# tobwei/APTAI

Measured on AMD Instinct MI355X. Metric: utterances/sec (10 s @ 16 kHz) train-step, higher is better.
Workload: dtype bf16

## Files before the change

### aptai_amd/csrc/gemm.hip

```cpp
#include <stdlib.h>

#include <mutex>
#include <set>
#include <type_traits>

#include "common.h"
#include "gemm_common.h"

using namespace aptai_gemm;

namespace {

#ifdef APTAI_STAMPS
__device__ unsigned long long g_stamps[4096 * 8];
#define APTAI_STAMP(slot)                                                                          \
    do {                                                                                           \
        if (threadIdx.x == 0 && blockIdx.x < 4096 && blockIdx.y == 0 && blockIdx.z == 0)           \
            g_stamps[blockIdx.x * 8 + (slot)] = wall_clock64();                                    \
    } while (0)
extern "C" int aptai_debug_read_stamps(void* host_out) {
    return hipMemcpyFromSymbol(host_out, HIP_SYMBOL(g_stamps), sizeof(g_stamps)) == hipSuccess ? 0 : 1;
}
#else
#define APTAI_STAMP(slot) do {} while (0)
#endif

void epi_trace(const GemmArgs& g, int tile) {
    static const bool on = getenv("APTAI_EPI_TRACE") != nullptr;
    if (!on) return;
    static std::mutex mu;
    static std::set<int> seen;
    const int w = g.flags | (g.out_pre ? EPX_PRE : 0) | (g.colscale_n > 0 ? EPX_CS : 0);
    std::lock_guard<std::mutex> lk(mu);
    if (!seen.insert(w).second) return;
    bool listed = false;
#define APTAI_EPI_CASE(W) listed = listed || (w == (W));
    APTAI_EPI_WORDS(APTAI_EPI_CASE)
#undef APTAI_EPI_CASE
    fprintf(stderr, "[aptai epi] flag word 0x%x (tile %d, %d x %d x %d): %s\n", w, tile, g.M, g.N, g.K, listed ? "compiled" : "RUN-TIME form");
}

template <bool A_KM, bool B_KM, bool OUT_F32, int BM_T = 128>
__device__ __forceinline__ void gemm_tile_body(GemmArgs g, const int bid, const int batch, const int split) {
    extern __shared__ __attribute__((aligned(16))) char smem[];
    APTAI_STAMP(0);
    const int tid = threadIdx.x;
    const int lane = tid & 63;
    const int wave = __builtin_amdgcn_readfirstlane(tid >> 6);
    const int wm = wave >> 1, wn = wave & 1;

    int tile_m, tile_n;
    raster2d(bid, g.tiles_m, g.tiles_n, g.raster_gm, tile_m, tile_n);
    constexpr int NI = BM_T / 32;
    constexpr int WM = BM_T / 2;
    constexpr int NA_IT = BM_T / 32;
    constexpr int A_BYTES_T = BM_T * BK * 2;
    constexpr int STAGE_T = A_BYTES_T + BN * BK * 2;
    constexpr int NPASS = BM_T / 16;
    static_assert(BM_T == 128 || (BM_T == 64 && !A_KM), "64-row tiles are built for K-contiguous A only");
    constexpr bool RING5 = A_KM && B_KM && BM_T == 128 && APTAI_GEMM_RING5;
    const int m0 = tile_m * BM_T, n0 = tile_n * BN;

    if (batch >= 0) {
        const int bo = batch / g.nb_inner, bi = batch % g.nb_inner;
        g.A += bo * g.sA[0] + bi * g.sA[1];
        g.B += bo * g.sB[0] + bi * g.sB[1];
        const long co = bo * g.sC[0] + bi * g.sC[1];
        g.C = (OUT_F32 && !(g.flags & APTAI_EPI_SPLIT_OUT)) ? (void*)((float*)g.C + co) : (void*)((bf16_t*)g.C + co);
        if (g.out_pre) g.out_pre += co;
        if (g.bias) g.bias += bo * g.sBias[0] + bi * g.sBias[1];
        if (g.residual) g.residual += bo * g.sR[0] + bi * g.sR[1];
        if (g.aux) g.aux += bo * g.sAux[0] + bi * g.sAux[1];
    }
    const int total_kt = g.K / BK;
    const int kt_begin = split * g.ktiles_per_split;
    int kt_end = kt_begin + g.ktiles_per_split;
    kt_end = kt_end < total_kt ? kt_end : total_kt;
    const int nk = kt_end - kt_begin;

    f32x4 acc[NI][4];
#pragma unroll
    for (int i = 0; i < NI; ++i)
#pragma unroll
        for (int j = 0; j < 4; ++j) acc[i][j] = (f32x4){0.f, 0.f, 0.f, 0.f};

    const int wave_base_tid = wave * 64;
    const bool wave_active = (m0 + wm * WM < g.M) && (n0 + wn * 64 < g.N);
    const bf16_t* pa[NA_IT];
    const bf16_t* pb[4];
    const long stepA = A_KM ? (long)BK * g.lda : (long)BK, stepB = B_KM ? (long)BK * g.ldb : (long)BK;
#pragma unroll
    for (int it = 0; it < NA_IT; ++it) pa[it] = stage_src<A_KM>(g.A, g.lda, m0, g.M, it, tid) + kt_begin * stepA;
#pragma unroll
    for (int it = 0; it < 4; ++it) pb[it] = stage_src<B_KM>(g.B, g.ldb, n0, g.N, it, tid) + kt_begin * stepB;
    auto stage = [&](char* buf) {
        char* dst = buf + wave_base_tid * 16;
#pragma unroll
        for (int it = 0; it < NA_IT; ++it) {
            __builtin_amdgcn_global_load_lds(GLB_PTR(pa[it]), LDS_PTR(dst + it * (NTHREADS * 16)), 16, 0, 0);
            pa[it] += stepA;
        }
#pragma unroll
        for (int it = 0; it < 4; ++it) {
            __builtin_amdgcn_global_load_lds(GLB_PTR(pb[it]), LDS_PTR(dst + A_BYTES_T + it * (NTHREADS * 16)), 16, 0, 0);
            pb[it] += stepB;
        }
    };
    if constexpr (RING5) {
        constexpr int HALF_T = RING_HALF_BYTES;
        const bf16_t* ha[2];
        const bf16_t* hb[2];
        const long hstepA = 32 * (long)g.lda, hstepB = 32 * (long)g.ldb;
#pragma unroll
        for (int it = 0; it < 2; ++it) {
            ha[it] = stage_src<true>(g.A, g.lda, m0, g.M, it, tid) + kt_begin * stepA;
            hb[it] = stage_src<true>(g.B, g.ldb, n0, g.N, it, tid) + kt_begin * stepB;
        }
        auto stage_half = [&](int slot) {
            char* dst = smem + slot * HALF_T + wave_base_tid * 16;
#pragma unroll
            for (int it = 0; it < 2; ++it) {
                __builtin_amdgcn_global_load_lds(GLB_PTR(ha[it]), LDS_PTR(dst + it * (NTHREADS * 16)), 16, 0, 0);
                ha[it] += hstepA;
            }
#pragma unroll
            for (int it = 0; it < 2; ++it) {
                __builtin_amdgcn_global_load_lds(GLB_PTR(hb[it]), LDS_PTR(dst + HALF_T / 2 + it * (NTHREADS * 16)), 16, 0, 0);
                hb[it] += hstepB;
            }
        };
        uint32_t frag_off[16];
        {
            const int gq = lane >> 4, li = lane & 15, qq = li >> 2, pp = li & 3;
            const int k_lo = gq * 8 + qq, k_hi = k_lo + 4;
            const int sub = (pp & 1) << 3;
#pragma unroll
            for (int f = 0; f < 8; ++f) {
                const int is_b = f >> 2, idx = f & 3;
                const int row_base = is_b ? wn * 64 + idx * 16 : wm * WM + idx * 16;
                const int ch = (row_base >> 3) + (pp >> 1);
                frag_off[2 * f] = (uint32_t)(is_b * (HALF_T / 2) + k_lo * 256 + ((ch ^ km_swz(k_lo)) << 4) + sub);
                frag_off[2 * f + 1] = (uint32_t)(is_b * (HALF_T / 2) + k_hi * 256 + ((ch ^ km_swz(k_hi)) << 4) + sub);
            }
        }
        const uint32_t ring_base = (uint32_t)(uintptr_t)(__attribute__((address_space(3))) const char*)smem;
        const int nh = 2 * nk;
        if (nh > 0) { stage_half(0); stage_half(1); }
        if (nh > 2) stage_half(2);
        int s0 = 0;
        for (int kt = 0; kt < nk; ++kt) {
            if (kt + 1 < nk) asm volatile("s_waitcnt vmcnt(4) lgkmcnt(0)" ::: "memory");
            else asm volatile("s_waitcnt vmcnt(0) lgkmcnt(0)" ::: "memory");
            __builtin_amdgcn_s_barrier();
            asm volatile("" ::: "memory");
            const int s1 = s0 + 1 >= 5 ? s0 - 4 : s0 + 1, s2 = s0 + 2 >= 5 ? s0 - 3 : s0 + 2, s3 = s0 + 3 >= 5 ? s0 - 2 : s0 + 3,
                      s4 = s0 + 4 >= 5 ? s0 - 1 : s0 + 4;
            if (2 * kt + 3 < nh) stage_half(s3);
            if (2 * kt + 4 < nh) stage_half(s4);
            if (wave_active) {
                short4v fr[2][16];
#pragma unroll
                for (int hh = 0; hh < 2; ++hh) {
                    const uint32_t base = ring_base + (uint32_t)((hh ? s1 : s0) * HALF_T);
#pragma unroll
                    for (int f = 0; f < 16; ++f)
                        asm volatile("ds_read_b64_tr_b16 %0, %1" : "=v"(fr[hh][f]) : "v"(base + frag_off[f]));
                }
#define APTAI_TIE8(h, o) "+v"(fr[h][o]), "+v"(fr[h][o + 1]), "+v"(fr[h][o + 2]), "+v"(fr[h][o + 3]), "+v"(fr[h][o + 4]), \
                         "+v"(fr[h][o + 5]), "+v"(fr[h][o + 6]), "+v"(fr[h][o + 7])
#pragma unroll
                for (int hh = 0; hh < 2; ++hh) {
                    if (hh == 0) asm volatile("s_waitcnt lgkmcnt(15)" : APTAI_TIE8(0, 0), APTAI_TIE8(0, 8));
                    else asm volatile("s_waitcnt lgkmcnt(0)" : APTAI_TIE8(1, 0), APTAI_TIE8(1, 8));
                    bf16x8 af[NI], bfr[4];
#pragma unroll
                    for (int i = 0; i < NI; ++i) {
                        const short4v lo4 = fr[hh][2 * i], hi4 = fr[hh][2 * i + 1];
                        af[i] = __builtin_bit_cast(bf16x8, (short8v){lo4[0], lo4[1], lo4[2], lo4[3], hi4[0], hi4[1], hi4[2], hi4[3]});
                    }
#pragma unroll
                    for (int j = 0; j < 4; ++j) {
                        const short4v lo4 = fr[hh][8 + 2 * j], hi4 = fr[hh][8 + 2 * j + 1];
                        bfr[j] = __builtin_bit_cast(bf16x8, (short8v){lo4[0], lo4[1], lo4[2], lo4[3], hi4[0], hi4[1], hi4[2], hi4[3]});
                    }
#pragma unroll
                    for (int i = 0; i < NI; ++i)
#pragma unroll
                        for (int j = 0; j < 4; ++j)
                            acc[i][j] = __builtin_amdgcn_mfma_f32_16x16x32_bf16(bfr[j], af[i], acc[i][j], 0, 0, 0);
                }
#undef APTAI_TIE8
            }
            s0 = s2;
        }
        asm volatile("s_waitcnt vmcnt(0) lgkmcnt(0)" ::: "memory");
        __syncthreads();
    } else {
    if (nk > 0) stage(smem);
    for (int kt = 0; kt < nk; ++kt) {
        asm volatile("s_waitcnt vmcnt(0)" ::: "memory");
        __syncthreads();
        const int cur = kt & 1;
        if (kt + 1 < nk) stage(smem + (cur ^ 1) * STAGE_T);
        const char* sa = smem + cur * STAGE_T;
        const char* sb = sa + A_BYTES_T;
        if (wave_active) {
            if constexpr (!A_KM && !B_KM && APTAI_GEMM_HOIST) {
                bf16x8 af[2][NI], bfr[2][4];
#pragma unroll
                for (int ks = 0; ks < 2; ++ks) {
#pragma unroll
                    for (int j = 0; j < 4; ++j) bfr[ks][j] = read_frag<B_KM>(sb, wn * 64 + j * 16, ks, lane);
#pragma unroll
                    for (int i = 0; i < NI; ++i) af[ks][i] = read_frag<A_KM>(sa, wm * WM + i * 16, ks, lane);
                }
                __builtin_amdgcn_sched_barrier(0);
#pragma unroll
                for (int ks = 0; ks < 2; ++ks)
#pragma unroll
                    for (int i = 0; i < NI; ++i)
#pragma unroll
                        for (int j = 0; j < 4; ++j)
                            acc[i][j] = __builtin_amdgcn_mfma_f32_16x16x32_bf16(bfr[ks][j], af[ks][i], acc[i][j], 0, 0, 0);
            } else if constexpr (BM_T == 64 && !A_KM && B_KM && APTAI_GEMM_M64_ASM) {
                short4v bl[2][4], bh[2][4];
                u32x4 aa[2][2];
#pragma unroll
                for (int ks = 0; ks < 2; ++ks) {
#pragma unroll
                    for (int j = 0; j < 4; ++j) read_frag_tr_asm(sb, wn * 64 + j * 16, ks, lane, bl[ks][j], bh[ks][j]);
#pragma unroll
                    for (int i = 0; i < 2; ++i) {
                        const int row = wm * WM + i * 16 + (lane & 15), q = ks * 4 + (lane >> 4);
                        const uint32_t addr = lds_u32(sa) + (uint32_t)(row * 128 + ((q ^ (row & 7)) << 4));
                        asm volatile("ds_read_b128 %0, %1" : "=v"(aa[ks][i]) : "v"(addr));
                    }
                }
#pragma unroll
                for (int ks = 0; ks < 2; ++ks) {
                    if (ks == 0)
                        asm volatile("s_waitcnt lgkmcnt(10)" : "+v"(bl[0][0]), "+v"(bl[0][1]), "+v"(bl[0][2]), "+v"(bl[0][3]), "+v"(bh[0][0]),
                                                               "+v"(bh[0][1]), "+v"(bh[0][2]), "+v"(bh[0][3]), "+v"(aa[0][0]), "+v"(aa[0][1]));
                    else
                        asm volatile("s_waitcnt lgkmcnt(0)" : "+v"(bl[1][0]), "+v"(bl[1][1]), "+v"(bl[1][2]), "+v"(bl[1][3]), "+v"(bh[1][0]),
                                                              "+v"(bh[1][1]), "+v"(bh[1][2]), "+v"(bh[1][3]), "+v"(aa[1][0]), "+v"(aa[1][1]));
#pragma unroll
                    for (int i = 0; i < 2; ++i)
#pragma unroll
                        for (int j = 0; j < 4; ++j)
                            acc[i][j] = __builtin_amdgcn_mfma_f32_16x16x32_bf16(combine_tr(bl[ks][j], bh[ks][j]),
                                                                                __builtin_bit_cast(bf16x8, aa[ks][i]), acc[i][j], 0, 0, 0);
                }
            } else {
#pragma unroll
                for (int ks = 0; ks < 2; ++ks) {
                    bf16x8 af[NI], bfr[4];
                    constexpr bool ASM_TR = BM_T == 128;
                    short4v tl[NI + 4], th[NI + 4];
#pragma unroll
                    for (int j = 0; j < 4; ++j) {
                        if constexpr (B_KM && ASM_TR) read_frag_tr_asm(sb, wn * 64 + j * 16, ks, lane, tl[NI + j], th[NI + j]);
                        else bfr[j] = read_frag<B_KM>(sb, wn * 64 + j * 16, ks, lane);
                    }
#pragma unroll
                    for (int i = 0; i < NI; ++i) {
                        if constexpr (A_KM && ASM_TR) read_frag_tr_asm(sa, wm * WM + i * 16, ks, lane, tl[i], th[i]);
                        else af[i] = read_frag<A_KM>(sa, wm * WM + i * 16, ks, lane);
                    }
                    if constexpr (B_KM && ASM_TR) {
                        asm volatile("s_waitcnt lgkmcnt(0)"
                                     : "+v"(tl[NI]), "+v"(tl[NI + 1]), "+v"(tl[NI + 2]), "+v"(tl[NI + 3]), "+v"(th[NI]), "+v"(th[NI + 1]),
                                       "+v"(th[NI + 2]), "+v"(th[NI + 3]));
#pragma unroll
                        for (int j = 0; j < 4; ++j) bfr[j] = combine_tr(tl[NI + j], th[NI + j]);
                    }
                    if constexpr (A_KM && ASM_TR) {
                        static_assert(!A_KM || NI == 4, "K-major A is built for 128-row tiles");
                        asm volatile("s_waitcnt lgkmcnt(0)"
                                     : "+v"(tl[0]), "+v"(tl[1]), "+v"(tl[2]), "+v"(tl[3]), "+v"(th[0]), "+v"(th[1]), "+v"(th[2]), "+v"(th[3]));
#pragma unroll
                        for (int i = 0; i < NI; ++i) af[i] = combine_tr(tl[i], th[i]);
                    }
#pragma unroll
                    for (int i = 0; i < NI; ++i)
#pragma unroll
                        for (int j = 0; j < 4; ++j)
                            acc[i][j] = __builtin_amdgcn_mfma_f32_16x16x32_bf16(bfr[j], af[i], acc[i][j], 0, 0, 0);
                }
            }
        }
    }
    }

    APTAI_STAMP(2);
    int tid_e = tid, lane_e = lane, m0_e = __builtin_amdgcn_readfirstlane(m0), n0_e = __builtin_amdgcn_readfirstlane(n0);
    asm volatile("" : "+v"(tid_e), "+v"(lane_e), "+s"(m0_e), "+s"(n0_e));
    const int fx = epi_flag_word(g);
    auto body = [&](auto w) {
        constexpr int FM = decltype(w)::value;
        const int flags = FM >= 0 ? FM : fx;
        const int cl = (tid_e & 15) * 8;
        const int n = n0_e + cl;
        const bool n_ok = n < g.N;
        constexpr bool PREF = !OUT_F32 && FM >= 0 && (FM & (APTAI_EPI_RESIDUAL | APTAI_EPI_DGELU | APTAI_EPI_MUL_AUX)) != 0;
        constexpr int NPF = PREF ? NPASS : 1;
        u32x4 resv[NPF], auxv[NPF];
#pragma unroll
        for (int pass = 0; pass < NPF; ++pass) {
            const int m = m0_e + pass * 16 + (tid_e >> 4);
            const bool ok = PREF && n_ok && m < g.M;
            u32x4 rq = {0u, 0u, 0u, 0u}, aq = {0u, 0u, 0u, 0u};
            if (ok && (flags & APTAI_EPI_RESIDUAL)) rq = *(const u32x4*)(g.residual + (long)m * g.ldr + n);
            if (ok && (flags & (APTAI_EPI_DGELU | APTAI_EPI_MUL_AUX))) aq = *(const u32x4*)(g.aux + (long)m * g.ldaux + n);
            resv[pass] = rq;
            auxv[pass] = aq;
        }
        __syncthreads();
        {
            char* ct = smem;
    #pragma unroll
            for (int i = 0; i < NI; ++i) {
                const int ml = wm * WM + i * 16 + (lane_e & 15);
    #pragma unroll
                for (int j = 0; j < 4; ++j) {
                    const int nl = wn * 64 + j * 16 + (lane_e >> 4) * 4;
                    *(f32x4*)(ct + ml * EPI_PITCH + nl * 4) = acc[i][j];
                }
            }
        }
        __syncthreads();
        float bias8[8];
    #pragma unroll
        for (int r = 0; r < 8; ++r) bias8[r] = 0.f;
        if ((flags & APTAI_EPI_BIAS) && n_ok) {
            const f32x4 b0 = *(const f32x4*)(g.bias + n), b1 = *(const f32x4*)(g.bias + n + 4);
    #pragma unroll
            for (int r = 0; r < 4; ++r) { bias8[r] = b0[r]; bias8[4 + r] = b1[r]; }
        }
        const float alpha = (flags & APTAI_EPI_ALPHA) ? g.alpha : 1.0f;
        uint32_t sd0 = g.seed0, sd1 = g.seed1;
        if (flags & APTAI_EPI_DROPOUT) apply_salt(g.salt, sd0, sd1);
        auto one_pass = [&](const int pass, const u32x4 auxq, const u32x4 resq) __attribute__((always_inline)) {
            const int ml = pass * 16 + (tid_e >> 4);
            const int m = m0_e + ml;
// ... 35 lines not shown
                if (ok && (flags & APTAI_EPI_RESIDUAL)) rq = *(const u32x4*)(g.residual + (long)m * g.ldr + n);
                if (ok && (flags & (APTAI_EPI_DGELU | APTAI_EPI_MUL_AUX))) aq = *(const u32x4*)(g.aux + (long)m * g.ldaux + n);
                one_pass(pass, aq, rq);
            }
        } else {
#pragma unroll
            for (int pass = 0; pass < NPASS; ++pass) {
                one_pass(pass, auxv[PREF ? pass : 0], resv[PREF ? pass : 0]);
                asm volatile("" ::: "memory");
            }
        }
    };
    if (OUT_F32) body(EpiWord<-1>{});
    else epi_dispatch(fx, body);
    APTAI_STAMP(3);
#ifdef APTAI_STAMPS
    asm volatile("s_waitcnt vmcnt(0)" ::: "memory");
    APTAI_STAMP(4);
#endif
}

template <bool A_KM, bool B_KM, bool OUT_F32>
__global__ __launch_bounds__(NTHREADS, 3) void gemm_kernel(GemmArgs g) {
#ifdef APTAI_EXP_STAGGER
    if (g.exp_sleep > 0) {
        bool late = true;
        if (g.exp_cu_count != nullptr) {
            unsigned hwid, xcc;
            asm volatile("s_getreg_b32 %0, hwreg(HW_REG_HW_ID)" : "=s"(hwid));
            asm volatile("s_getreg_b32 %0, hwreg(HW_REG_XCC_ID)" : "=s"(xcc));
            __shared__ unsigned arrival;
            if (threadIdx.x == 0) arrival = atomicAdd(g.exp_cu_count + ((xcc & 7u) * 256u + ((hwid >> 8) & 0xffu)), 1u);
            __syncthreads();
            late = arrival == 1u;
        }
        if (late) for (int i = 0; i < g.exp_sleep; ++i) __builtin_amdgcn_s_sleep(31);
    }
#endif
    gemm_tile_body<A_KM, B_KM, OUT_F32>(g, xcd_remap(blockIdx.x, g.tiles_m * g.tiles_n), gridDim.y > 1 ? (int)blockIdx.y : -1,
                                        blockIdx.z);
}

constexpr int SMEM_M64_BYTES = 2 * (64 + BN) * BK * 2;
template <bool B_KM, bool OUT_F32>
__global__ __launch_bounds__(NTHREADS, 3) void gemm_kernel_m64(GemmArgs g) {
    gemm_tile_body<false, B_KM, OUT_F32, 64>(g, xcd_remap(blockIdx.x, g.tiles_m * g.tiles_n), gridDim.y > 1 ? (int)blockIdx.y : -1,
                                             blockIdx.z);
}

constexpr int MAX_GROUP = 8;
struct GroupArgs {
    GemmArgs p[MAX_GROUP];
    int tile_end[MAX_GROUP];
    int n, total;
};

template <bool A_KM, bool B_KM, bool OUT_F32>
__global__ __launch_bounds__(NTHREADS, 3) void gemm_grouped_kernel(GroupArgs ga) {
    const int bid = xcd_remap(blockIdx.x, ga.total);
    int pi = 0;
#pragma unroll
    for (int i = 1; i < MAX_GROUP; ++i)
        if (i < ga.n && bid >= ga.tile_end[i - 1]) pi = i;
    const int first = pi ? ga.tile_end[pi - 1] : 0;
    gemm_tile_body<A_KM, B_KM, OUT_F32>(ga.p[pi], bid - first, -1, 0);
}

__global__ void splitk_reduce_kernel(const float* __restrict__ slabs, float* __restrict__ out, long n4, long slab_stride4,
                                     int nsplit, int accumulate) {
    const long stride = (long)gridDim.x * blockDim.x;
    for (long i = (long)blockIdx.x * blockDim.x + threadIdx.x; i < n4; i += stride) {
        f32x4 s = accumulate ? ((const f32x4*)out)[i] : (f32x4){0.f, 0.f, 0.f, 0.f};
        for (int k = 0; k < nsplit; ++k) s += ((const f32x4*)slabs)[(long)k * slab_stride4 + i];
        ((f32x4*)out)[i] = s;
    }
}

template <bool A_KM, bool B_KM, bool OUT_F32>
int launch_gemm128(const GemmArgs& g, dim3 grid, hipStream_t stream) {
    constexpr auto kern = gemm_kernel<A_KM, B_KM, OUT_F32>;
    constexpr int smem = smem_for<A_KM, B_KM>();
#ifdef APTAI_EXP_STAGGER
    {
        GemmArgs ge = g;
        const char* e = getenv("APTAI_EXP_SLEEP");
        ge.exp_sleep = e ? atoi(e) : 0;
        const char* c = getenv("APTAI_EXP_CU_COUNT");
        ge.exp_cu_count = c ? (unsigned*)(uintptr_t)strtoull(c, nullptr, 10) : nullptr;
        const char* m = getenv("APTAI_EXP_SMEM");
        const int sm = m ? atoi(m) : smem;
        (void)hipFuncSetAttribute((const void*)kern, hipFuncAttributeMaxDynamicSharedMemorySize, sm > smem ? sm : smem);
        APTAI_LAUNCH(kern, grid, dim3(NTHREADS), sm > smem ? sm : smem, stream, ge);
        APTAI_CHECK_LAUNCH("gemm_kernel");
        return APTAI_OK;
    }
#endif
    return launch_kernel<kern>({NTHREADS, smem, "gemm_kernel"}, grid, stream, g);
}


constexpr int T2_THREADS = 512;
constexpr int T2_BM = 256, T2_BN = 256;
constexpr int T2_HALF_BYTES = 128 * BK * 2;
constexpr int T2_BUF_BYTES = 4 * T2_HALF_BYTES;
constexpr int T2_SMEM = 2 * T2_BUF_BYTES;
static_assert(128 * T2_BN * 4 <= T2_SMEM, "an epilogue pass (128 fp32 rows, unpadded) must fit the staging LDS");

template <bool KM>
__device__ __forceinline__ void stage_half(const bf16_t* __restrict__ base, long ld, int row0, int rows_total, int k0,
                                           char* lds_half, int tid, int wave_base_tid) {
#pragma unroll
    for (int it = 0; it < 2; ++it) {
        const int cid = it * T2_THREADS + tid;
        const bf16_t* src;
        if (!KM) {
            const int row = cid >> 3, pc = cid & 7;
            int grow = row0 + row;
            grow = grow < rows_total ? grow : rows_total - 1;
// ... 962 lines not shown
}

static int launch_plan(const aptai_gemm_desc* d, const aptai_gemm_plan_info& p, void* stream_, long hash_ld, int hash_n0) {
    hipStream_t stream = (hipStream_t)stream_;
    GemmArgs g;
    fill_args(d, p, stream_, g);
    g.hash_ld = hash_ld; g.hash_n0 = hash_n0;
    if (gemm_knobs().epi_runtime) g.flags |= EPX_RUNTIME;
    const bool f32 = d->out_f32 != 0;
    if (!f32) epi_trace(g, p.tile);
    const dim3 grid(g.tiles_m * g.tiles_n, p.nbatch, p.nsplit);
    const int rc = with_layout("aptai_gemm_bf16", d->a_kmajor != 0, d->b_kmajor != 0, f32, [&](auto a, auto b, auto f) {
        constexpr bool A = a(), B = b(), F = f();
        switch (p.tile) {
        case 64: return launch_kernel<gemm_kernel_m64<B, F>>({NTHREADS, SMEM_M64_BYTES, "gemm_kernel_m64"}, grid, stream, g);
        case 192: return launch_kernel<gemm192_kernel<A, B, F>>({T3_THREADS, T3_SMEM, "gemm192_kernel"}, grid, stream, g);
        case 256: return launch_kernel<gemm256_kernel<A, B, F>>({T2_THREADS, T2_SMEM, "gemm256_kernel"}, grid, stream, g);
        case 257: return launch_gemm256_sk<A, B, F>(g, d->sk_workspace, stream);
        case 448: return launch_gemm_t4(g, B, stream);
        default: return launch_gemm128<A, B, F>(g, grid, stream);
        }
    });
    if (rc != APTAI_OK) return rc;
    if (f32 && (p.nsplit > 1 || d->accumulate)) {
        const long n4 = (long)d->M * d->N / 4;
        int blocks = (int)(n4 / 256 < 2048 ? (n4 + 255) / 256 : 2048);
        APTAI_LAUNCH(splitk_reduce_kernel, dim3(blocks), dim3(256), 0, stream, (const float*)d->workspace, (float*)d->C,
                           n4, g.slab_stride / 4, p.nsplit, d->accumulate ? 1 : 0);
        APTAI_CHECK_LAUNCH("splitk_reduce_kernel");
    }
    return APTAI_OK;
}

static int gemm_bf16_run(const aptai_gemm_desc* d, void* stream, long hash_ld, int hash_n0) {
    aptai_gemm_plan_info p;
    const int rc = aptai_gemm_plan(d, &p);
    if (rc != APTAI_OK) return rc;
    if (p.split_n == 0) return launch_plan(d, p, stream, hash_ld, hash_n0);
    const long n1 = p.split_n;
    aptai_gemm_desc a = *d, b = *d;
    a.N = n1; a.tile = 256;
    b.N = d->N - n1; b.tile = 128;
    b.B = (const char*)d->B + (d->b_kmajor ? n1 * 2 : n1 * d->ldb * 2);
    b.C = (char*)d->C + n1 * 2;
    if (d->out_pre) b.out_pre = (char*)d->out_pre + n1 * 2;
    if (d->bias) b.bias = d->bias + n1;
    if (d->residual) b.residual = (const char*)d->residual + n1 * 2;
    if (d->aux) b.aux = (const char*)d->aux + n1 * 2;
    const int rca = gemm_bf16_run(&a, stream, hash_ld, hash_n0);
    return rca != APTAI_OK ? rca : gemm_bf16_run(&b, stream, hash_ld, hash_n0 + (int)n1);
}
extern "C" int aptai_gemm_bf16(const aptai_gemm_desc* d, void* stream) { return gemm_bf16_run(d, stream, d ? d->N : 0, 0); }

extern "C" int aptai_gemm_bf16_grouped(const aptai_gemm_desc* descs, int n, void* stream_) {
    hipStream_t stream = (hipStream_t)stream_;
    APTAI_REQUIRE(descs != nullptr && n >= 1 && n <= MAX_GROUP, "aptai_gemm_bf16_grouped: need 1..%d problems, got %d", MAX_GROUP, n);
    GroupArgs ga;
    memset(&ga, 0, sizeof(ga));
    int total = 0;
    for (int i = 0; i < n; ++i) {
        const aptai_gemm_desc* d = descs + i;
        const int brc = validate_desc(d);
        if (brc != APTAI_OK) return brc;
        aptai_gemm_plan_info p = {};
        p.tile = 128;
        launch_shape(*d, p.nbatch, p.nsplit, p.ktiles_per_split);
        p.raster_gm = raster_group(gemm_knobs(), (d->a_kmajor && d->b_kmajor) ? 8 : 0);
        fill_args(d, p, stream_, ga.p[i]);
        APTAI_REQUIRE(p.nbatch == 1 && p.nsplit == 1 && !d->accumulate, "aptai_gemm_bf16_grouped: problem %d: no batching, split-K or accumulate", i);
        APTAI_REQUIRE(d->a_kmajor == descs[0].a_kmajor && d->b_kmajor == descs[0].b_kmajor && (d->out_f32 != 0) == (descs[0].out_f32 != 0),
                      "aptai_gemm_bf16_grouped: problem %d: all problems must share the operand layout and output type", i);
        total += ga.p[i].tiles_m * ga.p[i].tiles_n;
        ga.tile_end[i] = total;
    }
    ga.n = n;
    ga.total = total;
    return with_layout("aptai_gemm_bf16_grouped", descs[0].a_kmajor != 0, descs[0].b_kmajor != 0, descs[0].out_f32 != 0, [&](auto a, auto b, auto f) {
        return launch_kernel<gemm_grouped_kernel<a(), b(), f()>>({NTHREADS, smem_for<a(), b()>(), "gemm_grouped_kernel"}, dim3(total), stream, ga);
    });
}

extern "C" int64_t aptai_gemm_sk_workspace_bytes(void) { return sk_workspace_bytes(); }

extern "C" int aptai_gemm_sk_status(void* sk_workspace, void* stream, int* status_out) {
    APTAI_REQUIRE(sk_workspace != nullptr && status_out != nullptr, "aptai_gemm_sk_status: null pointer");
    unsigned v = 0;
    if (hipMemcpyAsync(&v, sk_workspace, 4, hipMemcpyDeviceToHost, (hipStream_t)stream) != hipSuccess ||
        hipStreamSynchronize((hipStream_t)stream) != hipSuccess)
        APTAI_FAIL(APTAI_ERR_LAUNCH, "aptai_gemm_sk_status: reading the status word failed");
    if (v != 0 && hipMemsetAsync(sk_workspace, 0, 4, (hipStream_t)stream) != hipSuccess)
        APTAI_FAIL(APTAI_ERR_LAUNCH, "aptai_gemm_sk_status: clearing the status word failed");
    *status_out = (int)v;
    return APTAI_OK;
}

extern "C" int64_t aptai_gemm_workspace_bytes(int64_t M, int64_t N, int split_k) {
    return (int64_t)(split_k > 0 ? split_k : 1) * M * N * 4;
}
```

### aptai_amd/ops.py

```python
from __future__ import annotations

import ctypes
from typing import Optional

import torch

from . import _lib

EPI_BIAS, EPI_GELU, EPI_RESIDUAL, EPI_DROPOUT, EPI_DGELU, EPI_ALPHA, EPI_PRE_DGELU, EPI_MUL_AUX, EPI_RESIDUAL_F32, EPI_SPLIT_OUT, EPI_BIAS_ROW = 1, 2, 4, 8, 16, 32, 64, 128, 256, 512, 1024

c_void_p, c_i64, c_int, c_float, c_u64 = (ctypes.c_void_p, ctypes.c_int64, ctypes.c_int, ctypes.c_float,
                                          ctypes.c_uint64)


class GemmDesc(ctypes.Structure):
    _fields_ = [("A", c_void_p), ("lda", c_i64), ("B", c_void_p), ("ldb", c_i64), ("C", c_void_p), ("ldc", c_i64),
                ("M", c_i64), ("N", c_i64), ("K", c_i64),
                ("a_kmajor", c_int), ("b_kmajor", c_int), ("out_f32", c_int), ("flags", c_int),
                ("bias", c_void_p), ("residual", c_void_p), ("ldr", c_i64), ("out_pre", c_void_p),
                ("aux", c_void_p), ("ldaux", c_i64), ("alpha", c_float), ("dropout_p", c_float), ("seed", c_u64),
                ("split_k", c_int), ("accumulate", c_int), ("workspace", c_void_p), ("workspace_bytes", c_i64),
                ("batch_outer", c_int), ("batch_inner", c_int),
                ("batch_stride_a", c_i64 * 2), ("batch_stride_b", c_i64 * 2), ("batch_stride_c", c_i64 * 2),
                ("batch_stride_bias", c_i64 * 2), ("batch_stride_res", c_i64 * 2), ("batch_stride_aux", c_i64 * 2),
# ... 140 lines not shown
    if batch is not None:
        d.batch_outer, d.batch_inner = batch.get("outer", 1), batch.get("inner", 1)
        for key, field in (("a", "batch_stride_a"), ("b", "batch_stride_b"), ("c", "batch_stride_c"),
                           ("bias", "batch_stride_bias"), ("res", "batch_stride_res"), ("aux", "batch_stride_aux")):
            so, si = batch.get(key, (0, 0))
            getattr(d, field)[0], getattr(d, field)[1] = so, si
    if out_f32 and (split_k > 1 or accumulate):
        need = _lib.lib().aptai_gemm_workspace_bytes(M, N, split_k)
        if workspace is None or workspace.numel() * workspace.element_size() < need:
            workspace = torch.empty(need, device=a.device, dtype=torch.uint8)
        d.workspace, d.workspace_bytes = workspace.data_ptr(), workspace.numel() * workspace.element_size()
    return out, workspace


_AUTO_TILE = 0


class auto_tile:

    def __init__(self, tile: int):
        self.tile = int(tile)

    def __enter__(self):
        global _AUTO_TILE
        self.prev, _AUTO_TILE = _AUTO_TILE, self.tile
        return self

    def __exit__(self, *exc):
        global _AUTO_TILE
        _AUTO_TILE = self.prev
        return False


def gemm(a: torch.Tensor, b: torch.Tensor, M: int, N: int, K: int, **kw) -> torch.Tensor:
    d = GemmDesc()
    out, _ws_keep = _gemm_desc(d, a, b, M, N, K, **kw)
    pr = _probe
    if pr is not None and pr.key == (bool(d.a_kmajor), bool(d.b_kmajor), bool(d.out_f32)) and not torch.cuda.is_current_stream_capturing():
        e0, e1 = torch.cuda.Event(enable_timing=True), torch.cuda.Event(enable_timing=True)
        e0.record()
        _lib.check(_lib.lib().aptai_gemm_bf16(ctypes.byref(d), c_void_p(_stream())), "aptai_gemm_bf16")
        e1.record()
        batch = kw.get("batch")
        nb = (batch.get("outer", 1) * batch.get("inner", 1)) if batch else 1
        pr.records.append((2.0 * M * N * K * nb, e0, e1))
        return out
    _lib.check(_lib.lib().aptai_gemm_bf16(ctypes.byref(d), c_void_p(_stream())), "aptai_gemm_bf16")
    return out


def gemm_grouped(problems) -> list:
    problems = list(problems)
    descs = (GemmDesc * len(problems))()
    outs, keep = [], []
    flops = 0.0
    for d, (a, b, M, N, K, kw) in zip(descs, problems):
        out, ws = _gemm_desc(d, a, b, M, N, K, **kw)
        outs.append(out)
        keep.append(ws)
        flops += 2.0 * M * N * K
    pr = _probe
    d0 = descs[0]
    if pr is not None and pr.key == (bool(d0.a_kmajor), bool(d0.b_kmajor), bool(d0.out_f32)) and not torch.cuda.is_current_stream_capturing():
        e0, e1 = torch.cuda.Event(enable_timing=True), torch.cuda.Event(enable_timing=True)
        e0.record()
        _lib.check(_lib.lib().aptai_gemm_bf16_grouped(descs, len(problems), c_void_p(_stream())), "aptai_gemm_bf16_grouped")
        e1.record()
        pr.records.append((flops, e0, e1))
        return outs
    _lib.check(_lib.lib().aptai_gemm_bf16_grouped(descs, len(problems), c_void_p(_stream())), "aptai_gemm_bf16_grouped")
    return outs


_ONES = {}


def ones_kmajor(K: int, device) -> torch.Tensor:
    key = (K, str(device))
    t = _ONES.get(key)
    if t is None:
        t = torch.ones((K, 8), device=device, dtype=torch.bfloat16)
        _ONES[key] = t
    return t


def mx_quantize(x: torch.Tensor, out=None):
    _dev(x)
    rows, K = x.shape
    if out is None:
        q = torch.empty((rows, K), device=x.device, dtype=torch.uint8)
        s = torch.empty((rows, K // 32), device=x.device, dtype=torch.uint8)
    else:
        q, s = out
    _lib.call("aptai_mx_quantize_bf16", x.data_ptr(), x.stride(0), q.data_ptr(), q.stride(0), s.data_ptr(), s.stride(0), rows, K, _stream())
    return q, s


def gemm_mxfp8(aq, a_s, bq, b_s, M, N, K, *, bias=None, gelu=False, residual=None, out=None):
    _dev(aq, a_s, bq, b_s, bias, residual, out)
    if out is None:
        out = torch.empty((M, N), device=aq.device, dtype=torch.bfloat16)
    _lib.call("aptai_gemm_mxfp8", aq.data_ptr(), a_s.data_ptr(), aq.stride(0), a_s.stride(0), bq.data_ptr(), b_s.data_ptr(), bq.stride(0),
              b_s.stride(0), out.data_ptr(), out.stride(0), _ptr(bias), int(gelu), _ptr(residual), residual.stride(0) if residual is not None else 0,
              M, N, K, _stream())
    return out


def layernorm_fwd_mx(x, gamma, beta, eps, *, want_bf16=False):
    _dev(x, gamma, beta)
    rows, cols = x.shape
    y = torch.empty_like(x) if want_bf16 else None
    q = torch.empty((rows, cols), device=x.device, dtype=torch.uint8)
    s = torch.empty((rows, cols // 32), device=x.device, dtype=torch.uint8)
    _lib.call("aptai_layernorm_fwd_mx", x.data_ptr(), gamma.data_ptr(), beta.data_ptr(), _ptr(y), q.data_ptr(), q.stride(0), s.data_ptr(), s.stride(0),
              rows, cols, eps, _stream())
    return y, q, s


def gemm_mxfp8_mxout(aq, a_s, bq, b_s, M, N, K, *, bias=None, gelu=False, out=None):
    _dev(aq, a_s, bq, b_s, bias)
    if out is None:
        q = torch.empty((M, N), device=aq.device, dtype=torch.uint8)
        s = torch.empty((M, N // 32), device=aq.device, dtype=torch.uint8)
    else:
# ... 818 lines not shown
```

### aptai_amd/wav2vec2.py

```python
from __future__ import annotations

import json
import math
import os
from types import SimpleNamespace
from typing import List, Optional, Tuple

import numpy as np
import torch
import torch.nn as nn

from . import hostlogic, ops
from .config import W2V2Config


def _round_up(x: int, m: int) -> int:
    return (x + m - 1) // m * m


def _rows_with_zero_slack(rows: int, C: int, dev, slack: int = 8) -> torch.Tensor:
    t = torch.empty((rows, C), device=dev, dtype=torch.bfloat16)
    t[rows - slack:].zero_()
    return t

# ... 173 lines not shown
        s1 = ops.gemm(ctx, w.wo, M, H, H, bias=w.bo, residual=x)
        if pre:
            ffn_in, fq, f_s = ops.layernorm_fwd_mx(s1, ln2w, ln2b, cfg.layer_norm_eps)
        else:
            ffn_in, fq, f_s = ops.layernorm_fwd_mx(s1, ln1w, ln1b, cfg.layer_norm_eps, want_bf16=True)
        hq, h_s = ops.gemm_mxfp8_mxout(fq, f_s, mx.w1[0], mx.w1[1], M, I, H, bias=w.b1, gelu=True)
        s2 = ops.gemm_mxfp8(hq, h_s, mx.w2[0], mx.w2[1], M, H, I, bias=w.b2, residual=s1 if pre else ffn_in)
        y = s2 if pre else ops.layernorm_fwd(s2, ln2w, ln2b, cfg.layer_norm_eps, save_stats=False)[0]
        return (y,), None

    def bwd(self, s, grads, x_needs):
        cfg, g, w = self.cfg, self.g, self.w
        M, H, I = g.M, cfg.hidden_size, cfg.intermediate_size
        heads = cfg.num_attention_heads
        p_h, p_a, p_att = s.p
        ln1w, ln1b, ln2w, ln2b = s.ln
        dprobs = grads[1] if len(grads) > 1 else None
        dy = grads[0].contiguous() if grads[0] is not None else torch.zeros_like(s.x)
        pre = cfg.do_stable_layer_norm
        if pre:
            ds2 = dy
            d_ffn_out = ops.dropout(ds2, p_h, _seed(self.seed, 4)) if p_h > 0 else ds2
            ffn_in = s.n2
        else:
            ds2, d_ffn_out, dg2, db2 = ops.layernorm_bwd(dy, s.s2, s.m2, s.r2, ln2w, dropout_p=p_h, seed=_seed(self.seed, 4))
            if d_ffn_out is None:
                d_ffn_out = ds2
            ffn_in = s.x1
        du = ops.gemm(d_ffn_out, w.w2, M, I, H, b_kmajor=True, mul_aux=s.u)
        if pre:
            dn2 = ops.gemm(du, w.w1, M, H, I, b_kmajor=True)
            ds1, d_att_out, dg2, db2 = ops.layernorm_bwd(dn2, s.s1, s.m2, s.r2, ln2w, dres=ds2, dropout_p=p_h,
                                                         seed=_seed(self.seed, 2))
        else:
            dx1 = ops.gemm(du, w.w1, M, H, I, b_kmajor=True, residual=ds2)
            ds1, d_att_out, dg1, db1 = ops.layernorm_bwd(dx1, s.s1, s.m1, s.r1, ln1w, dropout_p=p_h, seed=_seed(self.seed, 2))
        if d_att_out is None:
            d_att_out = ds1
        dctx = ops.gemm(d_att_out, w.wo, M, H, H, b_kmajor=True)
        st = self.attn_state
        dqkv = ops.attention_bwd(s.qkv, self.lens, s.ctx, dctx, s.lse, g.B, g.Tp, H, heads, q_prescaled=True, dropout_p=p_att,
                                 seed=_seed(self.seed, 1), dctx_zero_beyond_len=st is None or not st.seen)
        if dprobs is not None:
            ops.attention_probs_bwd(s.qkv, self.lens, s.lse[0], dprobs.contiguous(), g.B, g.Tp, H, heads, q_prescaled=True,
                                    dropout_p=p_att, seed=_seed(self.seed, 1), dqkv=dqkv)
            if st is not None:
                st.seen = True
        attn_in = s.n1 if pre else s.x
        if pre:
            dn1 = ops.gemm(dqkv, w.wqkv, M, H, 3 * H, b_kmajor=True)
            dx, _, dg1, db1 = ops.layernorm_bwd(dn1, s.x, s.m1, s.r1, ln1w, dres=ds1)
        else:
            dx = ops.gemm(dqkv, w.wqkv, M, H, 3 * H, b_kmajor=True, residual=ds1)
        tn = dict(a_kmajor=True, b_kmajor=True, out_f32=True)
        ones = ops.ones_kmajor(M, dy.device)
        dw2, dw1, dwo, dwqkv, r2, r1, ro, rq = ops.gemm_grouped([
            (d_ffn_out, s.hact, H, I, M, tn), (du, ffn_in, I, H, M, tn), (d_att_out, s.ctx, H, H, M, tn),
            (dqkv, attn_in, 3 * H, H, M, tn),
            (ones, d_ffn_out, 8, H, M, tn), (ones, du, 8, I, M, tn), (ones, d_att_out, 8, H, M, tn),
            (ones, dqkv, 8, 3 * H, M, tn)])
        dbias2, dbias1, dbo, dbqkv = r2[0], r1[0], ro[0], rq[0]
        return dx, (dg1, db1, dg2, db2, dwqkv[0:H], dwqkv[H:2 * H], dwqkv[2 * H:3 * H], dbqkv[0:H], dbqkv[H:2 * H],
                    dbqkv[2 * H:3 * H], dwo, dbo, dw1, dbias1, dw2, dbias2)


_SPEC_ON_DEVICE = os.environ.get("APTAI_SPEC_ON_DEVICE", "1") != "0"


class _FrontImpl:

    def __init__(self, cfg, geom, lens_i32, spec, training, seed, model):
        self.cfg, self.g, self.lens, self.spec, self.training, self.seed, self.model = cfg, geom, lens_i32, spec, training, seed, model

    def _packed(self, key, dev):
        cfg, g = self.cfg, self.g
        Cg = cfg.hidden_size // cfg.num_conv_pos_embedding_groups
        pad = cfg.num_conv_pos_embeddings // 2
        rows_p = g.Tp + 2 * pad
        n = cfg.num_conv_pos_embedding_groups * g.B * rows_p * Cg + Cg * 8
        buf = self.model._scratch(key, n, dev)
        return buf, rows_p, Cg, pad

    def _posconv_batch(self, Cg, rows_p, K, a_off=0):
        cfg, g = self.cfg, self.g
        G = cfg.num_conv_pos_embedding_groups
        H = cfg.hidden_size
        return dict(outer=g.B, inner=G, a=(rows_p * Cg, g.B * rows_p * Cg), b=(0, Cg * K), c=(g.Tp * H, Cg),
                    bias=(0, Cg), res=(g.Tp * H, Cg), aux=(g.Tp * H, Cg))

    def fwd(self, feats, params, need):
        cfg, g = self.cfg, self.g
        (fplw, fplb, pw, pb, embed, pcg, pcv, pcb, elw, elb) = params
        M, H, C = g.M, cfg.hidden_size, feats.shape[1]
        tr = self.training
        s = SimpleNamespace(feats=feats, params=params)
        s.n0, s.m0, s.r0 = ops.layernorm_fwd(feats, fplw, fplb, cfg.layer_norm_eps, save_stats=need)
        wp = self.model._cached(("proj",), [pw], lambda: ops.cast_bf16(pw))
        s.p_fp = cfg.feat_proj_dropout if tr else 0.0
        h0 = ops.gemm(s.n0, wp, M, H, C, bias=pb, dropout_p=s.p_fp, seed=_seed(self.seed, 11))
        ops.frame_mask_fwd(h0, self.lens, self.spec, embed, g.B, g.Tp, g.T, H)
        s.h0 = h0
        G, Kw = cfg.num_conv_pos_embedding_groups, cfg.num_conv_pos_embeddings
        xg, rows_p, Cg, pad = self._packed("pc_x", feats.device)
        ops.posconv_pack(h0, xg, g.B, g.Tp, H, G, pad)
        s.wf, s.wd, s.norm = self.model._cached(("posconv",), [pcg, pcv], lambda: ops.posconv_weight(pcv, pcg.reshape(-1), G))
        K = Kw * Cg
        s.u = torch.empty((M, H), device=feats.device, dtype=torch.bfloat16) if need else None
        s.s = torch.empty((M, H), device=feats.device, dtype=torch.bfloat16)
        if ops.posconv_kernel_fits(H, G, Kw):
            ops.posconv_gemm(xg, s.wf, s.s, g.B, g.Tp, H, G, Kw, pad, bias=pcb, gelu=True, residual=h0, out_pre=s.u)
        else:
            ops.gemm(xg, s.wf, g.Tp, Cg, K, lda=Cg, ldb=K, out=s.s, ldc=H, bias=pcb, gelu=True, residual=h0, ldr=H, out_pre=s.u,
                     batch=self._posconv_batch(Cg, rows_p, K))
        s.xg_key = "pc_x"
# ... 679 lines not shown
```

### include/aptai_hip.h

```cpp
#ifndef APTAI_HIP_H
#define APTAI_HIP_H
#include <stdint.h>

#ifdef __cplusplus
extern "C" {
#endif

typedef enum {
    APTAI_OK = 0,
    APTAI_ERR_INVALID = -1,
    APTAI_ERR_LAUNCH = -2,
    APTAI_ERR_NO_DEVICE = -3
} aptai_status;

const char* aptai_last_error(void);
int aptai_version(void);
int aptai_device_check(char* name, int name_len);
int aptai_set_seed_salt(void* stream, const void* device_ptr_2xu32);
int aptai_set_frame_bounds(void* stream, const void* device_ptr_2xi32);

enum {
    APTAI_EPI_BIAS = 1,
    APTAI_EPI_GELU = 2,
    APTAI_EPI_RESIDUAL = 4,
    APTAI_EPI_DROPOUT = 8,
    APTAI_EPI_DGELU = 16,
    APTAI_EPI_ALPHA = 32,
    APTAI_EPI_PRE_DGELU = 64,
    APTAI_EPI_MUL_AUX = 128,
    APTAI_EPI_RESIDUAL_F32 = 256,
    APTAI_EPI_BIAS_ROW = 1024,
    APTAI_EPI_SPLIT_OUT = 512
};

typedef struct {
    const void* A; int64_t lda;
    const void* B; int64_t ldb;
    void* C; int64_t ldc;
    int64_t M, N, K;
    int a_kmajor, b_kmajor, out_f32;
    int flags;
    const float* bias;
    const void* residual; int64_t ldr;
    void* out_pre;
    const void* aux; int64_t ldaux;
    float alpha;
    float dropout_p; uint64_t seed;
    int split_k;
    int accumulate;
    void* workspace; int64_t workspace_bytes;
    int batch_outer, batch_inner;
    int64_t batch_stride_a[2], batch_stride_b[2], batch_stride_c[2], batch_stride_bias[2], batch_stride_res[2],
        batch_stride_aux[2];
    int tile;
    int colscale_n; float colscale;
    void* sk_workspace;
    int64_t sk_workspace_bytes;
    int split_out_pieces;
    int split_out_bcol;
} aptai_gemm_desc;

int aptai_gemm_bf16(const aptai_gemm_desc* desc, void* stream);
int aptai_gemm_bf16_grouped(const aptai_gemm_desc* descs, int n, void* stream);
typedef struct {
    int tile;
    int nbatch, nsplit;
    int ktiles_per_split;
    int raster_gm;
    int64_t split_n;
} aptai_gemm_plan_info;
int aptai_gemm_plan(const aptai_gemm_desc* desc, aptai_gemm_plan_info* out);
int64_t aptai_gemm_workspace_bytes(int64_t M, int64_t N, int split_k);
int64_t aptai_gemm_sk_workspace_bytes(void);
int aptai_gemm_sk_status(void* sk_workspace, void* stream, int* status_out);

int aptai_split_f32(const float* x, int64_t ldx, int64_t rows, int64_t cols, int pattern, int pieces, int act, void* out, int64_t ldo,
                    void* stream);
int aptai_bias_act_res_f32(const float* x, int64_t ldx, const float* bias, const float* res, int64_t ldr, float* y, int64_t ldy,
                           int64_t rows, int64_t cols, int act, const int32_t* lens, int64_t rows_per_b, void* stream);
int aptai_softmax_rows_f32(float* s, const int32_t* lens, int64_t B, int64_t heads, int64_t Tp, void* stream);
int aptai_softmax_split_f32(const float* s, const int32_t* lens, int64_t B, int64_t heads, int64_t Tp, int pieces, void* out, int64_t ldo,
                            void* stream);
int aptai_attention_exact_fwd(const void* qkv_split, int64_t ld, const int32_t* lens, void* ctx_split, int64_t ldo, int64_t B, int64_t Tp,
                              int64_t H, int64_t heads, int pieces, float scale, void* stream);
int aptai_conv0_fwd_f32(const float* audio, int64_t B, int64_t S, const float* weight, const float* bias, const float* gamma,
                        const float* beta, int mode, float eps, float* out, int64_t T_real, int64_t T_alloc, const float* stats,
                        void* stream);
int aptai_conv0_fwd_split(const float* audio, int64_t B, int64_t S, const float* weight, const float* bias, const float* gamma,
                          const float* beta, int mode, float eps, void* out_split, int pieces, int64_t T_real, int64_t T_alloc,
                          const float* stats, void* stream);

int aptai_layernorm_fwd(const void* x, const float* gamma, const float* beta, void* y, float* mean, float* rstd,
                        int64_t rows, int64_t cols, float eps, int gelu_after, void* stream);
int aptai_layernorm_fwd_f32in(const float* x, const float* gamma, const float* beta, void* y_bf16, float* y_f32, int64_t rows,
                              int64_t cols, float eps, void* stream);
int aptai_layernorm_fwd_f32in_split(const float* x, const float* gamma, const float* beta, float* y_f32, void* y_split, int pieces,
                                    int64_t rows, int64_t cols, float eps, void* stream);
int aptai_layernorm_bwd(const void* dy, const void* x, const float* mean, const float* rstd, const float* gamma,
                        const void* dres, void* dx, void* dx_drop, float dropout_p, uint64_t seed, float* dgamma,
                        float* dbeta, void* workspace, int64_t rows, int64_t cols, const float* beta_if_gelu_after,
                        void* stream);
int64_t aptai_layernorm_bwd_workspace_bytes(int64_t rows, int64_t cols);
int aptai_layernorm_bwd_finalize_multi(const int64_t* table_dev, int64_t njobs, int64_t max_cols, void* stream);

int aptai_attention_fwd(const void* qkv, const int32_t* lens, void* ctx, float* lse2, float* ctx_f32, int64_t B, int64_t Tp,
                        int64_t H, int64_t heads, float scale, float dropout_p, uint64_t seed, int q_prescaled, void* stream);
int aptai_attention_bwd(const void* qkv, const int32_t* lens, const void* ctx, const float* ctx_f32, const void* dctx,
                        const float* lse2, float* delta_ws, void* dqkv, int64_t B, int64_t Tp, int64_t H, int64_t heads, float scale,
                        float dropout_p, uint64_t seed, int dctx_zero_beyond_len, int q_prescaled, void* stream);

int aptai_attention_probs_fwd(const void* qkv, const int32_t* lens, const float* lse2, float* probs, int64_t B, int64_t Tp, int64_t H,
                              int64_t heads, float scale, float dropout_p, uint64_t seed, int q_prescaled, void* stream);
int aptai_attention_probs_bwd(const void* qkv, const int32_t* lens, const float* lse2, const float* dprobs, float* rowsum_ws, void* dqkv,
                              int64_t B, int64_t Tp, int64_t H, int64_t heads, float scale, float dropout_p, uint64_t seed,
                              int q_prescaled, int accumulate, void* stream);

// ... 153 lines not shown
```

Before: 1739.

## Fuse bias-gradient row sums into grouped weight-gradient GEMM tiles

The four separate ones-vector GEMM problems that produced bias gradients are replaced by extra MFMAs against a constant ones fragment. These run inside the weight-gradient tiles of the first column-tile waves, and their results are written out as fp32 row sums. This removes the extra padded tiles that streamed every activation gradient over the full token dimension a second time. It adds an extra accumulator array and MFMAs to some waves. It also lowers the launch-bounds occupancy target to 2 for the K-major ring path, which may change register allocation and latency hiding.

```diff
diff --git a/aptai_amd/csrc/gemm.hip b/aptai_amd/csrc/gemm.hip
--- a/aptai_amd/csrc/gemm.hip
+++ b/aptai_amd/csrc/gemm.hip
@@ -40,8 +40,8 @@
     fprintf(stderr, "[aptai epi] flag word 0x%x (tile %d, %d x %d x %d): %s\n", w, tile, g.M, g.N, g.K, listed ? "compiled" : "RUN-TIME form");
 }
 
-template <bool A_KM, bool B_KM, bool OUT_F32, int BM_T = 128>
-__device__ __forceinline__ void gemm_tile_body(GemmArgs g, const int bid, const int batch, const int split) {
+template <bool A_KM, bool B_KM, bool OUT_F32, int BM_T = 128, bool ROWSUM = false>
+__device__ __forceinline__ void gemm_tile_body(GemmArgs g, const int bid, const int batch, const int split, float* rowsum = nullptr) {
     extern __shared__ __attribute__((aligned(16))) char smem[];
     APTAI_STAMP(0);
     const int tid = threadIdx.x;
@@ -83,6 +83,13 @@
     for (int i = 0; i < NI; ++i)
 #pragma unroll
         for (int j = 0; j < 4; ++j) acc[i][j] = (f32x4){0.f, 0.f, 0.f, 0.f};
+
+    static_assert(!ROWSUM || (A_KM && B_KM && OUT_F32 && BM_T == 128), "row sums ride on the K-major fp32 weight-gradient tile");
+    const bool rs_wave = ROWSUM && rowsum != nullptr && tile_n == 0 && wn == 0;
+    const bf16x8 ones8 = __builtin_bit_cast(bf16x8, (short8v){0x3f80, 0x3f80, 0x3f80, 0x3f80, 0x3f80, 0x3f80, 0x3f80, 0x3f80});
+    f32x4 racc[ROWSUM ? NI : 1];
+#pragma unroll
+    for (int i = 0; i < (ROWSUM ? NI : 1); ++i) racc[i] = (f32x4){0.f, 0.f, 0.f, 0.f};
 
     const int wave_base_tid = wave * 64;
     const bool wave_active = (m0 + wm * WM < g.M) && (n0 + wn * 64 < g.N);
@@ -188,6 +195,12 @@
 #pragma unroll
                         for (int j = 0; j < 4; ++j)
                             acc[i][j] = __builtin_amdgcn_mfma_f32_16x16x32_bf16(bfr[j], af[i], acc[i][j], 0, 0, 0);
+                    if constexpr (ROWSUM) {
+                        if (rs_wave) {
+#pragma unroll
+                            for (int i = 0; i < NI; ++i) racc[i] = __builtin_amdgcn_mfma_f32_16x16x32_bf16(ones8, af[i], racc[i], 0, 0, 0);
+                        }
+                    }
                 }
 #undef APTAI_TIE8
             }
@@ -286,10 +299,25 @@
 #pragma unroll
                         for (int j = 0; j < 4; ++j)
                             acc[i][j] = __builtin_amdgcn_mfma_f32_16x16x32_bf16(bfr[j], af[i], acc[i][j], 0, 0, 0);
+                    if constexpr (ROWSUM) {
+                        if (rs_wave) {
+#pragma unroll
+                            for (int i = 0; i < NI; ++i) racc[i] = __builtin_amdgcn_mfma_f32_16x16x32_bf16(ones8, af[i], racc[i], 0, 0, 0);
+                        }
+                    }
                 }
             }
         }
     }
+    }
+    if constexpr (ROWSUM) {
+        if (rs_wave && lane < 16) {
+#pragma unroll
+            for (int i = 0; i < NI; ++i) {
+                const int m = m0 + wm * WM + i * 16 + lane;
+                if (m < g.M) rowsum[m] = racc[i][0];
+            }
+        }
     }
 
     APTAI_STAMP(2);
@@ -431,18 +459,19 @@
 struct GroupArgs {
     GemmArgs p[MAX_GROUP];
     int tile_end[MAX_GROUP];
+    float* rowsum[MAX_GROUP];
     int n, total;
 };
 
 template <bool A_KM, bool B_KM, bool OUT_F32>
-__global__ __launch_bounds__(NTHREADS, 3) void gemm_grouped_kernel(GroupArgs ga) {
+__global__ __launch_bounds__(NTHREADS, (A_KM && B_KM && APTAI_GEMM_RING5) ? 2 : 3) void gemm_grouped_kernel(GroupArgs ga) {
     const int bid = xcd_remap(blockIdx.x, ga.total);
     int pi = 0;
 #pragma unroll
     for (int i = 1; i < MAX_GROUP; ++i)
         if (i < ga.n && bid >= ga.tile_end[i - 1]) pi = i;
     const int first = pi ? ga.tile_end[pi - 1] : 0;
-    gemm_tile_body<A_KM, B_KM, OUT_F32>(ga.p[pi], bid - first, -1, 0);
+    gemm_tile_body<A_KM, B_KM, OUT_F32, 128, A_KM && B_KM && OUT_F32>(ga.p[pi], bid - first, -1, 0, ga.rowsum[pi]);
 }
 
 __global__ void splitk_reduce_kernel(const float* __restrict__ slabs, float* __restrict__ out, long n4, long slab_stride4,
@@ -1511,7 +1540,7 @@
 }
 extern "C" int aptai_gemm_bf16(const aptai_gemm_desc* d, void* stream) { return gemm_bf16_run(d, stream, d ? d->N : 0, 0); }
 
-extern "C" int aptai_gemm_bf16_grouped(const aptai_gemm_desc* descs, int n, void* stream_) {
+extern "C" int aptai_gemm_bf16_grouped_rowsum(const aptai_gemm_desc* descs, float* const* rowsums, int n, void* stream_) {
     hipStream_t stream = (hipStream_t)stream_;
     APTAI_REQUIRE(descs != nullptr && n >= 1 && n <= MAX_GROUP, "aptai_gemm_bf16_grouped: need 1..%d problems, got %d", MAX_GROUP, n);
     GroupArgs ga;
@@ -1519,6 +1548,13 @@
     int total = 0;
     for (int i = 0; i < n; ++i) {
         const aptai_gemm_desc* d = descs + i;
+        if (rowsums != nullptr && rowsums[i] != nullptr) {
+            APTAI_REQUIRE(d->a_kmajor && d->b_kmajor, "aptai_gemm_bf16_grouped: problem %d: row sums need both operands K-major", i);
+            APTAI_REQUIRE(d->out_f32, "aptai_gemm_bf16_grouped: problem %d: row sums need fp32 output", i);
+            APTAI_REQUIRE(d->split_k <= 1, "aptai_gemm_bf16_grouped: problem %d: row sums cannot be split over K slabs (each slab would hold a partial sum)", i);
+            APTAI_REQUIRE((uintptr_t)rowsums[i] % 4 == 0, "aptai_gemm_bf16_grouped: problem %d: row sums must be 4-byte aligned", i);
+            ga.rowsum[i] = rowsums[i];
+        }
         const int brc = validate_desc(d);
         if (brc != APTAI_OK) return brc;
         aptai_gemm_plan_info p = {};
@@ -1539,6 +1575,10 @@
     });
 }
 
+extern "C" int aptai_gemm_bf16_grouped(const aptai_gemm_desc* descs, int n, void* stream) {
+    return aptai_gemm_bf16_grouped_rowsum(descs, nullptr, n, stream);
+}
+
 extern "C" int64_t aptai_gemm_sk_workspace_bytes(void) { return sk_workspace_bytes(); }
 
 extern "C" int aptai_gemm_sk_status(void* sk_workspace, void* stream, int* status_out) {
diff --git a/aptai_amd/ops.py b/aptai_amd/ops.py
--- a/aptai_amd/ops.py
+++ b/aptai_amd/ops.py
@@ -216,24 +216,42 @@
 def gemm_grouped(problems) -> list:
     problems = list(problems)
     descs = (GemmDesc * len(problems))()
-    outs, keep = [], []
+    outs, keep, sums = [], [], []
+    rs_ptrs = (c_void_p * len(problems))()
     flops = 0.0
-    for d, (a, b, M, N, K, kw) in zip(descs, problems):
+    for i, (d, (a, b, M, N, K, kw)) in enumerate(zip(descs, problems)):
+        kw = dict(kw)
+        want_sum = kw.pop("rowsum", False)
         out, ws = _gemm_desc(d, a, b, M, N, K, **kw)
         outs.append(out)
         keep.append(ws)
+        if want_sum is not False and want_sum is not None:
+            rs = want_sum if isinstance(want_sum, torch.Tensor) else torch.empty((M,), device=a.device, dtype=torch.float32)
+            _dev(rs)
+            if rs.dtype != torch.float32 or rs.numel() != M or not rs.is_contiguous():
+                raise ValueError("rowsum takes a contiguous fp32 tensor of M elements")
+            rs_ptrs[i] = rs.data_ptr()
+            sums.append(rs)
         flops += 2.0 * M * N * K
+
+    def launch():
+        if sums:
+            _lib.check(_lib.lib().aptai_gemm_bf16_grouped_rowsum(descs, rs_ptrs, len(problems), c_void_p(_stream())),
+                       "aptai_gemm_bf16_grouped_rowsum")
+        else:
+            _lib.check(_lib.lib().aptai_gemm_bf16_grouped(descs, len(problems), c_void_p(_stream())), "aptai_gemm_bf16_grouped")
+
     pr = _probe
     d0 = descs[0]
     if pr is not None and pr.key == (bool(d0.a_kmajor), bool(d0.b_kmajor), bool(d0.out_f32)) and not torch.cuda.is_current_stream_capturing():
         e0, e1 = torch.cuda.Event(enable_timing=True), torch.cuda.Event(enable_timing=True)
         e0.record()
-        _lib.check(_lib.lib().aptai_gemm_bf16_grouped(descs, len(problems), c_void_p(_stream())), "aptai_gemm_bf16_grouped")
+        launch()
         e1.record()
         pr.records.append((flops, e0, e1))
-        return outs
-    _lib.check(_lib.lib().aptai_gemm_bf16_grouped(descs, len(problems), c_void_p(_stream())), "aptai_gemm_bf16_grouped")
-    return outs
+        return outs + sums
+    launch()
+    return outs + sums
 
 
 _ONES = {}
diff --git a/aptai_amd/wav2vec2.py b/aptai_amd/wav2vec2.py
--- a/aptai_amd/wav2vec2.py
+++ b/aptai_amd/wav2vec2.py
@@ -249,14 +249,10 @@
             dx, _, dg1, db1 = ops.layernorm_bwd(dn1, s.x, s.m1, s.r1, ln1w, dres=ds1)
         else:
             dx = ops.gemm(dqkv, w.wqkv, M, H, 3 * H, b_kmajor=True, residual=ds1)
-        tn = dict(a_kmajor=True, b_kmajor=True, out_f32=True)
-        ones = ops.ones_kmajor(M, dy.device)
-        dw2, dw1, dwo, dwqkv, r2, r1, ro, rq = ops.gemm_grouped([
+        tn = dict(a_kmajor=True, b_kmajor=True, out_f32=True, rowsum=True)
+        dw2, dw1, dwo, dwqkv, dbias2, dbias1, dbo, dbqkv = ops.gemm_grouped([
             (d_ffn_out, s.hact, H, I, M, tn), (du, ffn_in, I, H, M, tn), (d_att_out, s.ctx, H, H, M, tn),
-            (dqkv, attn_in, 3 * H, H, M, tn),
-            (ones, d_ffn_out, 8, H, M, tn), (ones, du, 8, I, M, tn), (ones, d_att_out, 8, H, M, tn),
-            (ones, dqkv, 8, 3 * H, M, tn)])
-        dbias2, dbias1, dbo, dbqkv = r2[0], r1[0], ro[0], rq[0]
+            (dqkv, attn_in, 3 * H, H, M, tn)])
         return dx, (dg1, db1, dg2, db2, dwqkv[0:H], dwqkv[H:2 * H], dwqkv[2 * H:3 * H], dbqkv[0:H], dbqkv[H:2 * H],
                     dbqkv[2 * H:3 * H], dwo, dbo, dw1, dbias1, dw2, dbias2)
 
diff --git a/include/aptai_hip.h b/include/aptai_hip.h
--- a/include/aptai_hip.h
+++ b/include/aptai_hip.h
@@ -62,6 +62,7 @@
 
 int aptai_gemm_bf16(const aptai_gemm_desc* desc, void* stream);
 int aptai_gemm_bf16_grouped(const aptai_gemm_desc* descs, int n, void* stream);
+int aptai_gemm_bf16_grouped_rowsum(const aptai_gemm_desc* descs, float* const* rowsums, int n, void* stream);
 typedef struct {
     int tile;
     int nbatch, nsplit;
```

After: 1758 (median of 6 runs). 1.1% higher.
